# pauxy-qmc/pauxy

Measured on AMD Instinct MI355X. Metric: walker_steps_per_sec, higher is better.
Workload: dtype f64; 1 GPU; generic Cholesky AFQMC: Nbasis=100, Nchol=500, RHF trial 25+25 electrons, 256 walkers/GPU, dt=0.005, reortho/10, comb/5, energy/10 (BASELINE configs[2]); walkers_total=256, rng=device-philox, population_control=device comb (one rank)

## Files before the change

### pauxy_amd/csrc/k_fused.hip

```cpp
#include <cstdlib>
#include <type_traits>

#include "mfma_gemm_wg.h"
#include "greens_small.h"

#define PF_D 3
#ifndef PF_NW
#define PF_NW 8
#endif
#define PF_NT (64 * PF_NW)
#ifndef PF_LW
#define PF_LW PF_NW
#endif
#define PF_FPW (16 / PF_LW)

struct PropFusedArgs {
    int M, na, nb, nt, order;
    int vhs_upper;
    int same_b;
    int b_real;
    int rem4;
    int hyb;
    int symcols;
    int closed_try;
    int contig;
    const cplx *BH1;
    const cplx *vhs;
    cplx *phi;
    const int *alive;
    const void *zero16;
    unsigned long long *n_closed;
    int resident;
};

__device__ inline d2_t lds_read_c(unsigned addr) { return lds_read_b128(addr); }

template <int OFF> __device__ inline d2_t lds_read_off(unsigned addr) {
    d2_t v;
    asm volatile("ds_read_b128 %0, %1 offset:%2" : "=v"(v) : "v"(addr), "n"(OFF));
    return v;
}
__device__ __attribute__((always_inline)) inline d2_t lds_read_frag(unsigned base, int idx) {
    switch (idx) {
    case 0: return lds_read_off<0>(base);
    case 1: return lds_read_off<1024>(base);
    case 2: return lds_read_off<2048>(base);
    case 3: return lds_read_off<3072>(base);
    case 4: return lds_read_off<4096>(base);
    case 5: return lds_read_off<5120>(base);
    case 6: return lds_read_off<6144>(base);
    default: return lds_read_off<7168>(base);
    }
}

template <int OFF> __device__ inline double lds_read_re_off(unsigned addr) {
    double v;
    asm volatile("ds_read_b64 %0, %1 offset:%2" : "=v"(v) : "v"(addr), "n"(OFF));
    return v;
}
__device__ __attribute__((always_inline)) inline double lds_read_frag_re(unsigned base, int idx) {
    switch (idx) {
    case 0: return lds_read_re_off<0>(base);
    case 1: return lds_read_re_off<1024>(base);
    case 2: return lds_read_re_off<2048>(base);
    case 3: return lds_read_re_off<3072>(base);
    case 4: return lds_read_re_off<4096>(base);
    case 5: return lds_read_re_off<5120>(base);
    case 6: return lds_read_re_off<6144>(base);
    default: return lds_read_re_off<7168>(base);
    }
}

__device__ inline void lds_barrier() {
    asm volatile("s_waitcnt lgkmcnt(0)" ::: "memory");
    __builtin_amdgcn_s_barrier();
    asm volatile("" ::: "memory");
}

struct StepHandoverArgs {
    unsigned char *t0_next;
    int *ready;
    const double *B2;
    unsigned long long *n_handed;
    int consume;
    int produce;
};

#include "k_fused_closed.h"

template <bool NARROW, int FULL>
__global__ __launch_bounds__(PF_NT) void prop_fused_kernel(PropFusedArgs a) {
    extern __shared__ __align__(16) unsigned char smem[];
    constexpr bool MUL3 = false;
#define PF_LEAVE(stored_closed_) return
#define PF_HANDOVER
#define PF_RESIDENT(KS_) prop_closed_resident<KS_, MUL3>(a, smem, phi, vhs)
#include "k_fused_body.h"
#undef PF_RESIDENT
#undef PF_HANDOVER
#undef PF_LEAVE
}

template <bool NARROW, int FULL, bool TAIL, bool MUL3>
__global__ __launch_bounds__(PF_NT) void prop_fused_kernel(PropFusedArgs a, GreensArgs ga, WeightArgs wa, const double *psiB) {
    static_assert(TAIL && !NARROW && FULL == 7, "the tail rides on the full wide deal only");
    static_assert(!MUL3, "the 3-multiplication tail kernel takes the step hand-over: the overload below");
    extern __shared__ __align__(16) unsigned char smem[];
    bool stored_closed = false;
    do {
#define PF_LEAVE(stored_closed_) { stored_closed = (stored_closed_); break; }
#define PF_HANDOVER
#define PF_RESIDENT(KS_) prop_closed_resident<KS_, false>(a, smem, phi, vhs)
#include "k_fused_body.h"
#undef PF_RESIDENT
#undef PF_HANDOVER
#undef PF_LEAVE
    } while (0);
    asm volatile("s_waitcnt vmcnt(0) lgkmcnt(0)" ::: "memory");
    __syncthreads();
    int w = blockIdx.x;
    asm volatile("" : "+s"(w));
    greens_small_body<true, true>(ga, wa, w, smem, stored_closed);
}

template <bool NARROW, int FULL, bool TAIL, bool MUL3>
__global__ __launch_bounds__(PF_NT) void prop_fused_kernel(PropFusedArgs a, GreensArgs ga, WeightArgs wa, const double *psiB,
                                                           StepHandoverArgs ho) {
    static_assert(TAIL && !NARROW && FULL == 7 && MUL3, "the tail rides on the full wide deal only");
    extern __shared__ __align__(16) unsigned char smem[];
    bool stored_closed = false;
    EarlyTail early;
    early.on = false;
    do {
#define PF_LEAVE(stored_closed_) { stored_closed = (stored_closed_); break; }
#define PF_HANDOVER                                                                                           \
    if (ho.consume) {                                                                                         \
        handed = __builtin_amdgcn_readfirstlane(ho.ready[w]) != 0;                                            \
        if (handed && threadIdx.x == 0) { atomicAdd(a.n_closed, 1ULL); atomicAdd(ho.n_handed, 1ULL); }        \
    }
#define PF_RESIDENT(KS_)                                                                                      \
    do {                                                                                                      \
        if (psiB) prop_closed_resident<KS_, true, true>(a, smem, phi, vhs, psiB, &early, &ho, handed);        \
        else prop_closed_resident<KS_, true>(a, smem, phi, vhs);                                              \
    } while (0)
#include "k_fused_body.h"
#undef PF_RESIDENT
#undef PF_HANDOVER
#undef PF_LEAVE
    } while (0);
    if (ho.ready && threadIdx.x == 0) ho.ready[blockIdx.x] = (early.on && ho.produce) ? 1 : 0;
    asm volatile("s_waitcnt vmcnt(0) lgkmcnt(0)" ::: "memory");
    __syncthreads();
    int w = blockIdx.x;
    asm volatile("" : "+s"(w));
    greens_small_body<true, true, true>(ga, wa, w, smem, stored_closed, &early);
}

int k_prop_fused_supported(afq_handle *h) {
    return !h->vhs_diag && h->nv == 1 && h->M <= 104 && h->na <= 32 && h->nb <= 32 && h->nb > 0;
}

int k_prop_closed_resident(afq_handle *h) {
    return PF_NW == 8 && k_prop_fused_supported(h) && h->prop_closed_mode != 1 && h->bh1_same && h->bh1_real &&
           h->na == h->nb && h->na > 16 && h->na <= 32 && h->M > 96 && h->M <= 104 && h->exp_order > 0;
}

int k_step_fusion_shape(afq_handle *h) {
    if (!k_prop_closed_resident(h)) return 0;
    const size_t nmax = h->na, NCH = (h->M + 7) / 8;
    const size_t tail = sizeof(cplx) * (2 * (nmax * nmax + 2 * nmax) + ((2 * nmax + 3) / 4 + 1) + (size_t)h->M * h->nt);
    return tail <= NCH * 8192 + (size_t)PF_D * 16384;
}

int k_prop_fused(afq_handle *h, const GreensLaunch *tail, bool mul3) {
    PropFusedArgs a;
    a.M = h->M; a.na = h->na; a.nb = h->nb; a.nt = h->nt; a.order = h->exp_order;
    a.vhs_upper = h->vhs_upper ? 1 : 0;
    a.same_b = h->bh1_same ? 1 : 0;
    a.b_real = h->bh1_real ? 1 : 0;
    a.rem4 = (h->M > 96 && h->M <= 100) ? 1 : 0;
    a.hyb = 0;
    a.contig = 0; a.symcols = 0;
    if (a.rem4 && a.same_b && h->na > 16 && h->nb > 16 && h->nt > 48 && h->nt <= 56 && PF_NW == 8) {
        a.contig = 1;
        a.hyb = (h->nt - 48 + 3) / 4;
    }
    a.symcols = (a.contig && h->na == h->nb) ? 1 : 0;
    a.closed_try = 0;
    a.BH1 = h->BH1; a.vhs = h->vhs; a.phi = h->phi; a.alive = h->alive; a.zero16 = h->zero_page;
    a.n_closed = h->counters + 3;
    const int NCH = (h->M + 7) / 8;
    const size_t lds = (size_t)NCH * 8192 + (size_t)PF_D * 16384;
    static size_t lds_set[8][AFQ_MAX_DEVICES] = {{0}, {0}, {0}, {0}, {0}, {0}, {0}, {0}};
    const bool narrow = h->na <= 16 && h->nb <= 16;
    const bool early = tail && mul3 && h->step_tail_overlap && h->psiB_cT && k_prop_closed_resident(h) &&
                       tail->a.psi_real && tail->a.psi_closed && tail->a.psi_stride == 0 &&
                       (const void *)tail->a.psi == h->psiB_psi && (const void *)h->BH1 == h->psiB_bh1 &&
                       tail->a.gsum && tail->a.ghalf && !tail->a.oinv;
    const bool consumes = early && h->handover.current && h->handover.enabled && h->t0_next && h->t0_ready;
    h->handover.drop();
    const bool produces = early && h->step_handover && h->handover.enabled && h->B2 && (const void *)h->BH1 == h->b2_bh1;
    if (produces && (!h->t0_next || !h->t0_ready)) {
        AFQ_TRY(dev_alloc(h, LT_WALKERS, &h->t0_next, (size_t)h->nw * ((h->M + 3) / 4) * 2048, "step hand-over image"));
        AFQ_TRY(dev_alloc(h, LT_WALKERS, &h->t0_ready, (size_t)h->nw, "step hand-over flags"));
    }
    KernelTrace kt(h, AFQ_K_PROPAGATOR);
    {
        const int nrt_ = (h->M + 15) / 16, ct = (h->na + 15) / 16 + (h->nb + 15) / 16;
        const double ksteps = 2.0 * NCH;
        const double per_pass = ksteps * (2048.0 * (a.rem4 ? nrt_ - 1 : nrt_) * ct + 512.0 * (a.rem4 ? ct : 0));
        const double taylor_pass = a.contig ? ksteps * (2048.0 * (nrt_ - 1) * 3 + 512.0 * (nrt_ - 1) * a.hyb + 512.0 * 4) : per_pass;
        h->issued_flops[AFQ_K_PROPAGATOR] = (3.0 * h->exp_order * taylor_pass + 2.0 * (a.b_real ? 2.0 : 3.0) * per_pass) * h->nw;
        h->prop_issued_open = h->issued_flops[AFQ_K_PROPAGATOR] / h->nw;
        const int cta = (h->na + 15) / 16;
        const double closed_pass = ksteps * (2048.0 * (a.rem4 ? nrt_ - 1 : nrt_) * cta + 512.0 * (a.rem4 ? cta : 0));
        h->prop_issued_closed = 3.0 * h->exp_order * closed_pass + 2.0 * (a.b_real ? 2.0 : 3.0) * per_pass;
        if (k_prop_closed_resident(h)) {
            const double passes = (consumes ? 0.0 : 1.0) + 1.0 + (produces ? 1.0 : 0.0);
            h->prop_issued_closed = ((tail && mul3 ? 3.0 : 4.0) * h->exp_order + passes * 2.0) * ((h->M + 3) / 4) * 2048.0 * 7 * 2;
        }
        if (tail) {
            const double t16 = (h->na + 15) / 16, m16 = (h->M + 15) / 16;
            const double ks1 = 4.0 * (((h->M + 3) / 4 + 3) / 4), ks3 = (h->na + 3) / 4;
            const double spin = 2048.0 * (t16 * t16 * ks1 * (tail->a.psi_real ? 2.0 : 3.0) + t16 * m16 * ks3 * 3.0);
            h->prop_issued_open += 2.0 * spin;
            h->prop_issued_closed += (tail->a.psi_closed ? 1.0 : 2.0) * spin;
            if (early) h->prop_issued_closed += 2048.0 * (4.0 * ((h->M + 3) / 4) * 2.0 - t16 * t16 * ks1 * 2.0);
            h->issued_flops[AFQ_K_PROPAGATOR] = h->prop_issued_open * h->nw;
        }
    }
    const int nrt = (h->M + 15) / 16;
    const bool nofull = PF_NW != 8;
    const int full = nofull ? 0 : narrow ? (nrt == 6 ? 6 : 0) : (nrt >= 5 && h->na > 16 && h->nb > 16 ? nrt : 0);
    a.closed_try = (a.same_b && h->na == h->nb && h->exp_order > 0 && full != 0 && PF_NW == 8 &&
                    (!a.contig || a.symcols)) ? 1 : 0;
    a.resident = (a.closed_try && full == 7 && k_prop_closed_resident(h)) ? 1 : 0;
#define PF_LAUNCH_(NARROW_, FULL_, SLOT_)                                                                     \
    do {                                                                                                      \
        AFQ_HIP(h, afq_raise_lds((const void *)prop_fused_kernel<NARROW_, FULL_>, lds, lds_set[SLOT_]));      \
        AFQ_LAUNCH(h, (prop_fused_kernel<NARROW_, FULL_>), dim3(h->nw), dim3(PF_NT), lds, h->stream, a);      \
    } while (0)
    if (tail) {
        if (full != 7 || !a.resident || tail->lds > lds)
            AFQ_FAIL(h, AFQ_ESTATE, "internal: a Green's function tail on a propagator launch outside its shape class");
        if (mul3) {
            void (*const kern)(PropFusedArgs, GreensArgs, WeightArgs, const double *, StepHandoverArgs) =
                prop_fused_kernel<false, 7, true, true>;
            AFQ_HIP(h, afq_raise_lds((const void *)kern, lds, lds_set[6]));
            const double *psiB = early ? h->psiB_cT : nullptr;
            StepHandoverArgs ho;
            ho.t0_next = h->t0_next; ho.ready = h->t0_ready; ho.B2 = h->B2; ho.n_handed = h->counters + 9;
            ho.consume = consumes ? 1 : 0; ho.produce = produces ? 1 : 0;
            AFQ_LAUNCH(h, (prop_fused_kernel<false, 7, true, true>), dim3(h->nw), dim3(PF_NT), lds, h->stream, a, tail->a, tail->wa, psiB, ho);
        } else {
            const double *psiB = nullptr;
            void (*const kern)(PropFusedArgs, GreensArgs, WeightArgs, const double *) = prop_fused_kernel<false, 7, true, false>;
            AFQ_HIP(h, afq_raise_lds((const void *)kern, lds, lds_set[7]));
            AFQ_LAUNCH(h, (prop_fused_kernel<false, 7, true, false>), dim3(h->nw), dim3(PF_NT), lds, h->stream, a, tail->a, tail->wa, psiB);
        }
    }
    else if (narrow && full) PF_LAUNCH_(true, 6, 0);
    else if (narrow) PF_LAUNCH_(true, 0, 1);
    else if (full == 7) PF_LAUNCH_(false, 7, 2);
    else if (full == 6) PF_LAUNCH_(false, 6, 3);
    else if (full == 5) PF_LAUNCH_(false, 5, 4);
    else PF_LAUNCH_(false, 0, 5);
#undef PF_LAUNCH_
    AFQ_POST(h);
    if (produces) h->handover.produced();
    return AFQ_OK;
}
```

### pauxy_amd/csrc/k_fused_closed.h

```cpp
#pragma once

#define PCR_LDS(p) ((__attribute__((address_space(3))) unsigned char *)(p))

template <int KS, bool MUL3, bool EARLY = false>
__device__ __attribute__((always_inline)) inline void prop_closed_resident(const PropFusedArgs &a, unsigned char *smem_,
                                                                           cplx *phi, const cplx *vhs,
                                                                           const double *psiB = nullptr, EarlyTail *et = nullptr,
                                                                           const StepHandoverArgs *ho = nullptr, const bool handed_ = false) {
    auto *smem = PCR_LDS(smem_);
    const bool handed = EARLY && handed_;
    typedef __attribute__((address_space(3))) d2_t lds_d2;
    typedef __attribute__((address_space(3))) double lds_f64;
    const int tid = threadIdx.x, wave = __builtin_amdgcn_readfirstlane(tid >> 6);
    const int M = a.M, nt = a.nt, na = a.na;
    constexpr unsigned TB = KS * 2048;
    const bool mul = wave < 7;
    auto lane_id = [&]() __attribute__((always_inline)) -> int {
        int t = tid;
        asm volatile("" : "+v"(t));
        return t & 63;
    };

    const unsigned base0 = (EARLY && (a.order & 1)) ? TB : 0u;
    constexpr int NCP = (KS * 128 + PF_NT - 1) / PF_NT;
    d2_t cp[NCP];
    if (handed) {
        const d2_t *t0 = (const d2_t *)(ho->t0_next + (size_t)blockIdx.x * TB);
#pragma unroll
        for (int i = 0; i < NCP; ++i) {
            const int e = tid + i * PF_NT;
            cp[i] = t0[e < KS * 128 ? e : 0];
        }
    } else {
        for (int e = tid; e < KS * 128; e += PF_NT) {
            const int k = 4 * (e >> 7) + ((e >> 4) & 3), col = 16 * ((e >> 6) & 1) + (e & 15);
            const bool ok = k < M && col < na;
            const cplx v = phi[ok ? k * nt + col : 0];
            ((lds_d2 *)(smem + base0))[e] = ok ? (d2_t){v.x, v.y} : (d2_t){0.0, 0.0};
        }
        __syncthreads();
    }

    auto load_b = [&](double (&bh)[KS]) __attribute__((always_inline)) {
        const int lane = lane_id(), lk = lane >> 4, row = wave * 16 + (lane & 15);
#pragma unroll
        for (int s = 0; s < KS; ++s) {
            const int k = 4 * s + lk;
            const double *p = (row < M && k < M) ? &a.BH1[row * M + k].x : (const double *)a.zero16;
            bh[s] = *p;
        }
    };
    auto one_body = [&](const unsigned src, const double (&bh)[KS], d4_t (&P1)[2], d4_t (&P2)[2]) __attribute__((always_inline)) {
#pragma unroll
        for (int j = 0; j < 2; ++j) { P1[j] = (d4_t){0, 0, 0, 0}; P2[j] = (d4_t){0, 0, 0, 0}; }
        const auto *tb = smem + src + lane_id() * 16;
#pragma unroll
        for (int s = 0; s < KS; ++s) {
#pragma unroll
            for (int j = 0; j < 2; ++j) {
                const d2_t b = *(const lds_d2 *)(tb + (s * 2 + j) * 1024);
                P1[j] = mfma16(bh[s], b[0], P1[j]);
                P2[j] = mfma16(bh[s], b[1], P2[j]);
            }
        }
    };
    auto put = [&](const unsigned dst, const d4_t (&re)[2], const d4_t (&im)[2]) __attribute__((always_inline)) {
        auto *tb = smem + dst + lane_id() * 16;
#pragma unroll
        for (int q = 0; q < 4; ++q)
            if (4 * wave + q < KS) {
#pragma unroll
                for (int j = 0; j < 2; ++j) *(lds_d2 *)(tb + ((4 * wave + q) * 2 + j) * 1024) = (d2_t){re[j][q], im[j][q]};
            }
    };

    d2_t av[KS];
    d4_t SR[2], SI[2];
    if (mul) {
        double bh[KS];
        if (handed) {
            const d2_t *t0 = (const d2_t *)(ho->t0_next + (size_t)blockIdx.x * TB) + lane_id();
#pragma unroll
            for (int q = 0; q < 4; ++q)
#pragma unroll
                for (int j = 0; j < 2; ++j) {
                    const d2_t v = 4 * wave + q < KS ? t0[((4 * wave + q) * 2 + j) * 64] : (d2_t){0.0, 0.0};
                    SR[j][q] = v[0]; SI[j][q] = v[1];
                }
        } else {
            load_b(bh);
        }
        const int lane = lane_id(), lk = lane >> 4, row = wave * 16 + (lane & 15);
#pragma unroll
        for (int s = 0; s < KS; ++s) {
            const int k = 4 * s + lk;
            const int off = (a.vhs_upper && k < row) ? k * M + row : row * M + k;
            const d2_t *p = (row < M && k < M) ? (const d2_t *)(vhs + off) : (const d2_t *)a.zero16;
            av[s] = *p;
        }
        if (!handed) {
            one_body(base0, bh, SR, SI);
            put(base0 ^ TB, SR, SI);
        }
    }
    constexpr unsigned PB = 2 * TB;
    if constexpr (EARLY) {
        if (!mul) {
            const int lane = lane_id(), lk = lane >> 4, lr = lane & 15;
            double pv[2][KS];
#pragma unroll
            for (int t = 0; t < 2; ++t)
#pragma unroll
                for (int s = 0; s < KS; ++s) {
                    const int j = 16 * t + lr, k = 4 * s + lk;
                    const double *p = (j < na && k < M) ? psiB + j * M + k : (const double *)a.zero16;
                    pv[t][s] = *p;
                }
            auto *pb = smem + PB + lane * 8;
#pragma unroll
            for (int t = 0; t < 2; ++t)
#pragma unroll
                for (int s = 0; s < KS; ++s) *(lds_f64 *)(pb + (t * KS + s) * 512) = pv[t][s];
        }
    }
    if (handed) {
#pragma unroll
        for (int i = 0; i < NCP; ++i) {
            const int e = tid + i * PF_NT;
            if (e < KS * 128) ((lds_d2 *)(smem + (base0 ^ TB)))[e] = cp[i];
        }
    }
    lds_barrier();

    unsigned cur = base0 ^ TB;
    for (int n = 1; n <= a.order; ++n) {
        if (mul) {
            double inv_n = 1.0 / n;
            asm volatile("" : "+v"(inv_n));
            d4_t P1[2], P2[2], P3[2];
#pragma unroll
            for (int j = 0; j < 2; ++j) { P1[j] = (d4_t){0, 0, 0, 0}; P2[j] = (d4_t){0, 0, 0, 0}; P3[j] = (d4_t){0, 0, 0, 0}; }
            const auto *tb = smem + cur + lane_id() * 16;
#pragma unroll
            for (int s = 0; s < KS; ++s) {
                asm volatile("" : "+v"(av[s]));
#pragma unroll
                for (int j = 0; j < 2; ++j) {
                    const d2_t b = *(const lds_d2 *)(tb + (s * 2 + j) * 1024);
                    if constexpr (MUL3) {
                        P1[j] = mfma16(av[s][0], b[0], P1[j]);
                        P2[j] = mfma16(av[s][1], b[1], P2[j]);
                        P3[j] = mfma16(av[s][0] + av[s][1], b[0] + b[1], P3[j]);
                    } else {
                        P3[j] = mfma16(av[s][0], b[1], P3[j]);
                        P1[j] = mfma16(av[s][0], b[0], P1[j]);
                        P2[j] = mfma16(av[s][1], b[1], P2[j]);
                        P3[j] = mfma16(av[s][1], b[0], P3[j]);
                    }
                }
            }
            d4_t re[2], im[2];
#pragma unroll
            for (int j = 0; j < 2; ++j)
#pragma unroll
                for (int q = 0; q < 4; ++q) {
                    re[j][q] = (P1[j][q] - P2[j][q]) * inv_n;
                    im[j][q] = (MUL3 ? P3[j][q] - P1[j][q] - P2[j][q] : P3[j][q]) * inv_n;
                    SR[j][q] += re[j][q]; SI[j][q] += im[j][q];
                }
            if (n == a.order) put(cur ^ TB, SR, SI);
            else put(cur ^ TB, re, im);
        }
        lds_barrier();
        cur ^= TB;
    }

    if constexpr (EARLY) {
        const int nn = na, nsq = nn * nn + 2 * nn;
        cplx *O = (cplx *)smem_;
        cplx *phi_l = (cplx *)smem_ + 2L * nsq + ((2 * nn + 3) / 4 + 1);
        {
            const int t = wave >> 2, j = (wave >> 1) & 1, part = wave & 1;
            const auto *pa = smem + PB + t * (KS * 512) + lane_id() * 8;
            const auto *tb = smem + cur + j * 1024 + part * 8 + lane_id() * 16;
            d4_t acc0 = {0, 0, 0, 0}, acc1 = {0, 0, 0, 0};
#pragma unroll
            for (int s = 0; s < KS; ++s) {
                const double x = *(const lds_f64 *)(pa + s * 512), y = *(const lds_f64 *)(tb + s * 2048);
                if (s & 1) acc1 = mfma16(x, y, acc1);
                else acc0 = mfma16(x, y, acc0);
            }
            const int lane = lane_id(), lr = lane & 15, lk = lane >> 4;
#pragma unroll
            for (int q = 0; q < 4; ++q) {
                const int i = 16 * j + lr, jj = 16 * t + 4 * q + lk;
                if (i < nn && jj < nn) ((double *)&O[i * nn + jj])[part] = acc0[q] + acc1[q];
            }
        }
        lds_barrier();
        d4_t P1[2], P2[2];
        if (mul) {
            double bh[KS];
            load_b(bh);
            one_body(cur, bh, P1, P2);
            const int lane = lane_id(), lr = lane & 15, lk = lane >> 4;
#pragma unroll
            for (int j = 0; j < 2; ++j)
#pragma unroll
                for (int q = 0; q < 4; ++q) {
                    const int orow = wave * 16 + lk + 4 * q, col = 16 * j + lr;
                    if (orow < M && col < na) {
                        const cplx v = cmake(P1[j][q], P2[j][q]);
                        phi[(long)orow * nt + col] = v;
                        phi[(long)orow * nt + na + col] = v;
                    }
                }
            if (ho->produce && wave != 3) {
                const bool third = wave == 4 || wave == 5;
                auto load_b2 = [&](const int rt, double (&bf)[KS]) __attribute__((always_inline)) {
                    const int ln = lane_id(), hk = ln >> 4, hrow = rt * 16 + (ln & 15);
#pragma unroll
                    for (int s = 0; s < KS; ++s) {
                        const int k = 4 * s + hk;
                        const double *p = (hrow < M && k < M) ? ho->B2 + hrow * M + k : (const double *)a.zero16;
                        bf[s] = *p;
                    }
                };
                auto store_t0 = [&](const int rt, const int j, const d4_t &re, const d4_t &im) __attribute__((always_inline)) {
                    d2_t *t0 = (d2_t *)(ho->t0_next + (size_t)blockIdx.x * TB) + lane_id();
#pragma unroll
                    for (int q = 0; q < 4; ++q)
                        if (4 * rt + q < KS) t0[((4 * rt + q) * 2 + j) * 64] = (d2_t){re[q], im[q]};
                };
                d4_t Q1[2], Q2[2];
                load_b2(wave, bh);
                if (third) {
                    double b3[KS];
                    load_b2(3, b3);
                    const int j3 = wave - 4;
                    d4_t X1 = {0, 0, 0, 0}, X2 = {0, 0, 0, 0};
#pragma unroll
                    for (int j = 0; j < 2; ++j) { Q1[j] = (d4_t){0, 0, 0, 0}; Q2[j] = (d4_t){0, 0, 0, 0}; }
                    const auto *tb = smem + cur + lane_id() * 16;
                    const auto *tx = tb + j3 * 1024;
#pragma unroll
                    for (int s = 0; s < KS; ++s) {
#pragma unroll
                        for (int j = 0; j < 2; ++j) {
                            const d2_t b = *(const lds_d2 *)(tb + (s * 2 + j) * 1024);
                            Q1[j] = mfma16(bh[s], b[0], Q1[j]);
                            Q2[j] = mfma16(bh[s], b[1], Q2[j]);
                        }
                        const d2_t b = *(const lds_d2 *)(tx + s * 2048);
                        X1 = mfma16(b3[s], b[0], X1);
                        X2 = mfma16(b3[s], b[1], X2);
                    }
                    store_t0(3, j3, X1, X2);
                } else {
                    one_body(cur, bh, Q1, Q2);
                }
#pragma unroll
                for (int j = 0; j < 2; ++j) store_t0(wave, j, Q1[j], Q2[j]);
            }
        } else {
            cplx *scr = O + nsq;
            gj_wave32(O, nn, lane_id(), true, scr, scr + 32, (int *)(scr + 64), et->ph, et->la);
        }
        lds_barrier();
        if (mul) {
            const int lane = lane_id(), lr = lane & 15, lk = lane >> 4;
#pragma unroll
            for (int j = 0; j < 2; ++j)
#pragma unroll
                for (int q = 0; q < 4; ++q) {
                    const int orow = wave * 16 + lk + 4 * q, col = 16 * j + lr;
                    if (orow < M && col < na) {
                        const cplx v = cmake(P1[j][q], P2[j][q]);
                        phi_l[orow * nt + col] = v;
                        phi_l[orow * nt + na + col] = v;
                    }
                }
        }
        et->on = true;
        return;
    }
    if (mul) {
        d4_t P1[2], P2[2];
        double bh[KS];
        load_b(bh);
        one_body(cur, bh, P1, P2);
        const int lane = lane_id(), lr = lane & 15, lk = lane >> 4;
#pragma unroll
        for (int j = 0; j < 2; ++j)
#pragma unroll
            for (int q = 0; q < 4; ++q) {
                const int orow = wave * 16 + lk + 4 * q, col = 16 * j + lr;
                if (orow < M && col < na) {
                    const cplx v = cmake(P1[j][q], P2[j][q]);
                    phi[(long)orow * nt + col] = v;
                    phi[(long)orow * nt + na + col] = v;
                }
            }
    }
}
```

Before: 1.210 million walker-steps/s.

## Use idle eighth wave to compute half of three waves' Taylor-series products

In the resident closed-shell propagation kernel with the 3-multiplication path, the eighth wave used to sit idle during the Taylor expansion loop. It now takes the upper half of the K range for the second column block of waves 4-6 and writes partial products to a new LDS region. Those waves add the partials in after an extra barrier. This balances MFMA work across all 8 waves at the cost of an extra LDS barrier per order and extra LDS space, guarded by a new size check.

```diff
diff --git a/pauxy_amd/csrc/k_fused.hip b/pauxy_amd/csrc/k_fused.hip
--- a/pauxy_amd/csrc/k_fused.hip
+++ b/pauxy_amd/csrc/k_fused.hip
@@ -161,6 +161,8 @@
 }
 
 int k_prop_closed_resident(afq_handle *h) {
+    const size_t KS = (h->M + 3) / 4, NCH = (h->M + 7) / 8;
+    if (KS * (2 * 2048 + 1024) + 3 * 4096 > NCH * 8192 + (size_t)PF_D * 16384) return 0;
     return PF_NW == 8 && k_prop_fused_supported(h) && h->prop_closed_mode != 1 && h->bh1_same && h->bh1_real &&
            h->na == h->nb && h->na > 16 && h->na <= 32 && h->M > 96 && h->M <= 104 && h->exp_order > 0;
 }
diff --git a/pauxy_amd/csrc/k_fused_closed.h b/pauxy_amd/csrc/k_fused_closed.h
--- a/pauxy_amd/csrc/k_fused_closed.h
+++ b/pauxy_amd/csrc/k_fused_closed.h
@@ -15,6 +15,10 @@
     const int M = a.M, nt = a.nt, na = a.na;
     constexpr unsigned TB = KS * 2048;
     const bool mul = wave < 7;
+    constexpr int KH = (KS + 1) / 2, KU = KS - KH;
+    constexpr unsigned PB = 2 * TB;
+    constexpr unsigned PP = PB + KS * 1024;
+    static_assert(PP + 3 * 4096 <= 13 * 8192 + PF_D * 16384, "the partial products lie inside the launch's LDS (M > 96)");
     auto lane_id = [&]() __attribute__((always_inline)) -> int {
         int t = tid;
         asm volatile("" : "+v"(t));
@@ -74,22 +78,69 @@
             }
     };
 
+    auto open_owner = [&](d2_t (&av)[KS], d4_t (&SR)[2], d4_t (&SI)[2]) __attribute__((always_inline)) {
+        auto load_v = [&]() __attribute__((always_inline)) {
+            const int lane = lane_id(), lk = lane >> 4, row = wave * 16 + (lane & 15);
+#pragma unroll
+            for (int s = 0; s < KS; ++s) {
+                const int k = 4 * s + lk;
+                const int off = (a.vhs_upper && k < row) ? k * M + row : row * M + k;
+                const d2_t *p = (row < M && k < M) ? (const d2_t *)(vhs + off) : (const d2_t *)a.zero16;
+                av[s] = *p;
+            }
+        };
+        if (handed) {
+            const d2_t *t0 = (const d2_t *)(ho->t0_next + (size_t)blockIdx.x * TB) + lane_id();
+#pragma unroll
+            for (int q = 0; q < 4; ++q)
+#pragma unroll
+                for (int j = 0; j < 2; ++j) {
+                    const d2_t v = 4 * wave + q < KS ? t0[((4 * wave + q) * 2 + j) * 64] : (d2_t){0.0, 0.0};
+                    SR[j][q] = v[0]; SI[j][q] = v[1];
+                }
+            load_v();
+        } else {
+            double bh[KS];
+            load_b(bh);
+            load_v();
+            one_body(base0, bh, SR, SI);
+            put(base0 ^ TB, SR, SI);
+        }
+    };
+    auto stage_psib = [&]() __attribute__((always_inline)) {
+        const int lane = lane_id(), lk = lane >> 4, lr = lane & 15;
+        double pv[2][KS];
+#pragma unroll
+        for (int t = 0; t < 2; ++t)
+#pragma unroll
+            for (int s = 0; s < KS; ++s) {
+                const int j = 16 * t + lr, k = 4 * s + lk;
+                const double *p = (j < na && k < M) ? psiB + j * M + k : (const double *)a.zero16;
+                pv[t][s] = *p;
+            }
+        auto *pb = smem + PB + lane * 8;
+#pragma unroll
+        for (int t = 0; t < 2; ++t)
+#pragma unroll
+            for (int s = 0; s < KS; ++s) *(lds_f64 *)(pb + (t * KS + s) * 512) = pv[t][s];
+    };
+    auto copy_t0 = [&]() __attribute__((always_inline)) {
+        if (handed) {
+#pragma unroll
+            for (int i = 0; i < NCP; ++i) {
+                const int e = tid + i * PF_NT;
+                if (e < KS * 128) ((lds_d2 *)(smem + (base0 ^ TB)))[e] = cp[i];
+            }
+        }
+    };
+    unsigned cur = base0 ^ TB;
+    if constexpr (!MUL3) {
+    static_assert(MUL3 || !EARLY, "the early tail and the hand-over belong to the 3-multiplication tail kernel");
     d2_t av[KS];
     d4_t SR[2], SI[2];
     if (mul) {
         double bh[KS];
-        if (handed) {
-            const d2_t *t0 = (const d2_t *)(ho->t0_next + (size_t)blockIdx.x * TB) + lane_id();
-#pragma unroll
-            for (int q = 0; q < 4; ++q)
-#pragma unroll
-                for (int j = 0; j < 2; ++j) {
-                    const d2_t v = 4 * wave + q < KS ? t0[((4 * wave + q) * 2 + j) * 64] : (d2_t){0.0, 0.0};
-                    SR[j][q] = v[0]; SI[j][q] = v[1];
-                }
-        } else {
-            load_b(bh);
-        }
+        load_b(bh);
         const int lane = lane_id(), lk = lane >> 4, row = wave * 16 + (lane & 15);
 #pragma unroll
         for (int s = 0; s < KS; ++s) {
@@ -98,41 +149,10 @@
             const d2_t *p = (row < M && k < M) ? (const d2_t *)(vhs + off) : (const d2_t *)a.zero16;
             av[s] = *p;
         }
-        if (!handed) {
-            one_body(base0, bh, SR, SI);
-            put(base0 ^ TB, SR, SI);
-        }
-    }
-    constexpr unsigned PB = 2 * TB;
-    if constexpr (EARLY) {
-        if (!mul) {
-            const int lane = lane_id(), lk = lane >> 4, lr = lane & 15;
-            double pv[2][KS];
-#pragma unroll
-            for (int t = 0; t < 2; ++t)
-#pragma unroll
-                for (int s = 0; s < KS; ++s) {
-                    const int j = 16 * t + lr, k = 4 * s + lk;
-                    const double *p = (j < na && k < M) ? psiB + j * M + k : (const double *)a.zero16;
-                    pv[t][s] = *p;
-                }
-            auto *pb = smem + PB + lane * 8;
-#pragma unroll
-            for (int t = 0; t < 2; ++t)
-#pragma unroll
-                for (int s = 0; s < KS; ++s) *(lds_f64 *)(pb + (t * KS + s) * 512) = pv[t][s];
-        }
-    }
-    if (handed) {
-#pragma unroll
-        for (int i = 0; i < NCP; ++i) {
-            const int e = tid + i * PF_NT;
-            if (e < KS * 128) ((lds_d2 *)(smem + (base0 ^ TB)))[e] = cp[i];
-        }
+        one_body(base0, bh, SR, SI);
+        put(base0 ^ TB, SR, SI);
     }
     lds_barrier();
-
-    unsigned cur = base0 ^ TB;
     for (int n = 1; n <= a.order; ++n) {
         if (mul) {
             double inv_n = 1.0 / n;
@@ -147,16 +167,10 @@
 #pragma unroll
                 for (int j = 0; j < 2; ++j) {
                     const d2_t b = *(const lds_d2 *)(tb + (s * 2 + j) * 1024);
-                    if constexpr (MUL3) {
-                        P1[j] = mfma16(av[s][0], b[0], P1[j]);
-                        P2[j] = mfma16(av[s][1], b[1], P2[j]);
-                        P3[j] = mfma16(av[s][0] + av[s][1], b[0] + b[1], P3[j]);
-                    } else {
-                        P3[j] = mfma16(av[s][0], b[1], P3[j]);
-                        P1[j] = mfma16(av[s][0], b[0], P1[j]);
-                        P2[j] = mfma16(av[s][1], b[1], P2[j]);
-                        P3[j] = mfma16(av[s][1], b[0], P3[j]);
-                    }
+                    P3[j] = mfma16(av[s][0], b[1], P3[j]);
+                    P1[j] = mfma16(av[s][0], b[0], P1[j]);
+                    P2[j] = mfma16(av[s][1], b[1], P2[j]);
+                    P3[j] = mfma16(av[s][1], b[0], P3[j]);
                 }
             }
             d4_t re[2], im[2];
@@ -165,7 +179,7 @@
 #pragma unroll
                 for (int q = 0; q < 4; ++q) {
                     re[j][q] = (P1[j][q] - P2[j][q]) * inv_n;
-                    im[j][q] = (MUL3 ? P3[j][q] - P1[j][q] - P2[j][q] : P3[j][q]) * inv_n;
+                    im[j][q] = P3[j][q] * inv_n;
                     SR[j][q] += re[j][q]; SI[j][q] += im[j][q];
                 }
             if (n == a.order) put(cur ^ TB, SR, SI);
@@ -173,6 +187,116 @@
         }
         lds_barrier();
         cur ^= TB;
+    }
+    } else {
+    auto kstep = [&](const d2_t &v, const unsigned char __attribute__((address_space(3))) *b_, d4_t &p1, d4_t &p2, d4_t &p3)
+        __attribute__((always_inline)) {
+        const d2_t b = *(const lds_d2 *)b_;
+        p1 = mfma16(v[0], b[0], p1);
+        p2 = mfma16(v[1], b[1], p2);
+        p3 = mfma16(v[0] + v[1], b[0] + b[1], p3);
+    };
+    auto owners = [&](auto whole_) __attribute__((always_inline)) {
+        constexpr bool WHOLE = decltype(whole_)::value;
+        d2_t av[KS];
+        d4_t SR[2], SI[2];
+        open_owner(av, SR, SI);
+        copy_t0();
+        lds_barrier();
+        for (int n = 1; n <= a.order; ++n) {
+            double inv_n = 1.0 / n;
+            asm volatile("" : "+v"(inv_n));
+            d4_t P1[2], P2[2], P3[2];
+#pragma unroll
+            for (int j = 0; j < 2; ++j) { P1[j] = (d4_t){0, 0, 0, 0}; P2[j] = (d4_t){0, 0, 0, 0}; P3[j] = (d4_t){0, 0, 0, 0}; }
+            const auto *tb = smem + cur + lane_id() * 16;
+#pragma unroll
+            for (int s = 0; s < KS; ++s) {
+                asm volatile("" : "+v"(av[s]));
+#pragma unroll
+                for (int j = 0; j < ((WHOLE || s < KH) ? 2 : 1); ++j) kstep(av[s], tb + (s * 2 + j) * 1024, P1[j], P2[j], P3[j]);
+                if (!WHOLE && (s & 3) == 3) __builtin_amdgcn_sched_barrier(0);
+            }
+            d4_t re[2], im[2];
+#pragma unroll
+            for (int j = 0; j < 2; ++j)
+#pragma unroll
+                for (int q = 0; q < 4; ++q) {
+                    re[j][q] = P1[j][q] - P2[j][q];
+                    im[j][q] = P3[j][q] - P1[j][q] - P2[j][q];
+                }
+            auto finish = [&]() __attribute__((always_inline)) {
+#pragma unroll
+                for (int j = 0; j < 2; ++j)
+#pragma unroll
+                    for (int q = 0; q < 4; ++q) {
+                        re[j][q] *= inv_n;
+                        im[j][q] *= inv_n;
+                        SR[j][q] += re[j][q]; SI[j][q] += im[j][q];
+                    }
+                if (n == a.order) put(cur ^ TB, SR, SI);
+                else put(cur ^ TB, re, im);
+            };
+            if constexpr (WHOLE) finish();
+            lds_barrier();
+            if constexpr (!WHOLE) {
+                const auto *pp = smem + PP + (wave - 4) * 4096 + lane_id() * 16;
+#pragma unroll
+                for (int q = 0; q < 4; ++q) {
+                    const d2_t u = *(const lds_d2 *)(pp + q * 1024);
+                    re[1][q] += u[0];
+                    im[1][q] += u[1];
+                }
+                finish();
+            }
+            lds_barrier();
+            cur ^= TB;
+        }
+    };
+    if (wave < 4) {
+        owners(std::true_type());
+    } else if (mul) {
+        owners(std::false_type());
+    } else {
+        if constexpr (EARLY) stage_psib();
+        copy_t0();
+        d2_t av7[3][KU];
+        asm volatile("" ::: "memory");
+        {
+            const int lane = lane_id(), lk = lane >> 4;
+#pragma unroll
+            for (int u = 0; u < 3; ++u)
+#pragma unroll
+                for (int i = 0; i < KU; ++i) {
+                    const int row = (4 + u) * 16 + (lane & 15), k = 4 * (KH + i) + lk;
+                    const int off = (a.vhs_upper && k < row) ? k * M + row : row * M + k;
+                    const d2_t *p = (row < M && k < M) ? (const d2_t *)(vhs + off) : (const d2_t *)a.zero16;
+                    av7[u][i] = *p;
+                }
+        }
+        lds_barrier();
+        for (int n = 1; n <= a.order; ++n) {
+            const auto *tb = smem + cur + 1024 + lane_id() * 16;
+            auto *pp = smem + PP + lane_id() * 16;
+#pragma unroll
+            for (int u = 0; u < 3; ++u) {
+                d4_t Q1 = {0, 0, 0, 0}, Q2 = {0, 0, 0, 0}, Q3 = {0, 0, 0, 0};
+#pragma unroll
+                for (int i = 0; i < KU; ++i) {
+                    asm volatile("" : "+v"(av7[u][i]));
+                    kstep(av7[u][i], tb + (KH + i) * 2048, Q1, Q2, Q3);
+                    if ((i & 3) == 3) __builtin_amdgcn_sched_barrier(0);
+                }
+#pragma unroll
+                for (int q = 0; q < 4; ++q)
+                    *(lds_d2 *)(pp + u * 4096 + q * 1024) = (d2_t){Q1[q] - Q2[q], Q3[q] - Q1[q] - Q2[q]};
+                __builtin_amdgcn_sched_barrier(0);
+            }
+            lds_barrier();
+            lds_barrier();
+            cur ^= TB;
+        }
+    }
     }
 
     if constexpr (EARLY) {
```

After: 1.232 million walker-steps/s, median of 6. 1.8% higher.
